# Antibas/eaQHM-analysis-and-synthesis-in-Python

Hardware: AMD Instinct MI355X
Metric: analysis_frames_per_sec (higher is better)
Workload: dtype f64; 1 GPU; synth16k_60s_female_maxAdpt5; samples=960000, fs=16000, ls_frames_per_adaptation=63936, adaptations_executed=5, Kmax=59, track_bytes=906240000, parallelism=instants sharded x1 by LS cost; boundary records all-gathered per adaptation

## Files before the change

eaqhm-analysis-and-synthesis-in-python_amd/csrc/eaqhm_ls_tile.hip:

```cpp
#include <type_traits>
#include "eaqhm_ls_common.h"
#include "eaqhm_ls_chol.h"
#include "eaqhm_ls_a0.h"
#include "eaqhm_ls_tilemap.h"
#include "eaqhm_ls_twunits.h"
#include "eaqhm_ls_gather.h"
#include "eaqhm_ls_tilelds.h"
#include "eaqhm_ls_tilexch.h"

namespace eaqhm {
bool ls_a0tile_fits(const LsArgs& A);
int launch_ls_a0tile(eaqhm_ctx* ctx, LsArgs A);

#define DIAG_OWNER(jb, nt) ((int)TL_DIAG[nt][jb])
#define TL_THREADS 512
#define TL_WAVES 8
#define TL_CW 8
static_assert(TLL_TILE == TL_TILE && TLL_DG_TILE == DG_TILE, "eaqhm_ls_tilelds.h and eaqhm_ls_chol.h disagree");
static_assert(TX_DFLAG_BYTE == 8 * (4 * TL_NTMAX * TL_TILE + 2 * TL_TILE + DGP_DOUBLES + 128 + 256), "eaqhm_ls_tilexch.h: where tile_frame puts dflag");

__device__ inline void fetch_next_header(const LsArgs& A, TlHead* hd, int C, int nbuf, int lane) {
  int* cls = uni(A.cls);
  int item = 0;
  if (lane == 0) item = atomicAdd(cls + 8 + C, 1);
  item = uni(item);
  int f = -1;
  if (item < uni(cls[C])) f = uni(cls[16 + (size_t)C * uni(A.n_frames) + item]);
  if (f >= 0) {
    const int* tab = (lane == 0) ? A.ncol : (lane == 1) ? A.frame_c : (lane == 2) ? A.frame_wl : A.frame_inst;
    if (lane < 4) (&hd->n)[lane] = tab[f];
    const int Kmax = uni(A.Kmax);
    if (lane < TL_NSLOT && lane < Kmax) hd->cols[nbuf][lane] = A.cols[(size_t)f * Kmax + lane];
  }
  if (lane == 0) { hd->f = f; hd->buf = nbuf; hd->cls = C; }
}

__device__ inline void tw_step(d4 (&g)[9], double aR, double aI, double bR, double bI, double nk) {
  const double sA = aR + aI, dB = bI - bR;
  const double naR = nk * aR, naI = nk * aI, nsA = nk * sA;
  const double nbR = nk * bR, nbI = nk * bI, ndB = nk * dB;
  g[0] = __builtin_amdgcn_mfma_f64_16x16x4f64(aR, bR, g[0], 0, 0, 0);
  g[1] = __builtin_amdgcn_mfma_f64_16x16x4f64(aI, bI, g[1], 0, 0, 0);
// ... 45 lines not shown
  g0[0] = __builtin_amdgcn_mfma_f64_16x16x4f64(aR, bR, g0[0], 0, 0, 0);
  g1[0] = __builtin_amdgcn_mfma_f64_16x16x4f64(aR, nbR, g1[0], 0, 0, 0);
  g0[1] = __builtin_amdgcn_mfma_f64_16x16x4f64(aR, bI, g0[1], 0, 0, 0);
  g1[1] = __builtin_amdgcn_mfma_f64_16x16x4f64(aR, nbI, g1[1], 0, 0, 0);
  g0[0] = __builtin_amdgcn_mfma_f64_16x16x4f64(aI, bI, g0[0], 0, 0, 0);
  g1[0] = __builtin_amdgcn_mfma_f64_16x16x4f64(aI, nbI, g1[0], 0, 0, 0);
  g0[1] = __builtin_amdgcn_mfma_f64_16x16x4f64(maI, bR, g0[1], 0, 0, 0);
  g1[1] = __builtin_amdgcn_mfma_f64_16x16x4f64(maI, nbR, g1[1], 0, 0, 0);
}

template <int NS, int TW, int UA = 0, int UB = 0, int TB = 0>
__device__ __attribute__((noinline)) void tile_frame(const LsArgs& A, int TS_, int ldx_max_, double* lds, int f_) {
  constexpr int C = NS == 12 ? 5 : NS == 10 ? 4 : NS == 9 ? 3 : NS == 7 ? 2 : NS == 6 ? 1 : 0;
  static_assert(NS == 12 || NS == 10 || NS == 9 || NS == 7 || NS == 6 || NS == 5, "a register budget per class");
  constexpr bool NEXT_HEAD = NS != 10, REC_ROW = NS == 9;
  const bool pre = uni(f_) < 0;
  const int TS = uni(TS_), ldx_max = uni(ldx_max_);
  const int tid = threadIdx.x, nt_thr = TL_THREADS;
  const int lane = tid & 63;
  const int wave = __builtin_amdgcn_readfirstlane(tid >> 6);
  double* U = uni(lds);
  TlHead* hd = (TlHead*)(U + tl_head_offset());
  const int f = pre ? uni(hd->f) : uni(f_);
  double* Xre = U;
  double* Xim = Xre + (size_t)TS * ldx_max;
  const size_t usize_g = (size_t)2 * TS * ldx_max;
  double* ci = U + usize_g;
  unsigned long long* masks = (unsigned long long*)(ci + (size_t)CI_STRIDE * 52);
  double* PanR = U;
  double* PanI = PanR + TL_NTMAX * TL_TILE;
  double* WtR = PanI + TL_NTMAX * TL_TILE;
  double* WtI = WtR + TL_NTMAX * TL_TILE;
  double* LdR = WtI + TL_NTMAX * TL_TILE;
  double* LdI = LdR + TL_TILE;
  double* Dc = LdI + TL_TILE;
  double* Zc = Dc + DG_TILE;
  double* zv = Zc + DG_TILE;
  double* xv = zv + 2 * 16 * TL_NTMAX;
  double* xs = xv + 32 + TL_HEAD_DOUBLES;
  double* sh = xs + 4 * uni(A.Kcmax);
  double* win = sh + 16;
  double* sig = win + 64 * CI_NCH;
  double* dorig = sig + 64 * CI_NCH;

  const int Npad = ((uni(A.Nmax) + 63) >> 6) << 6;
  double* Qs = uni(A.scratch) + (size_t)blockIdx.x * (size_t)uni((int)A.scratch_stride);
  double* Rs = Qs + (size_t)Npad * uni(A.nmax);
  const bool seeds = uni(hd->seeds) != 0;
  const double w1 = uni(2.0 * M_PI / A.fs);
  const int PE = TS / 2;
  const double* sA = uni(A.s);
  const int lcol = lane & 15, lq = lane >> 4;
  unsigned long long* dbg = uni(A.debug);
  unsigned long long t_prev = 0;

  {
    const int n = pre ? uni(hd->n) : uni(A.ncol[f]);
    const int Kc = 2 * n + 1, Ms = 2 * Kc + 1;
    const int nt = (Ms + 15) >> 4;
    const int c = pre ? uni(hd->c) : uni(A.frame_c[f]), wl = pre ? uni(hd->wl) : uni(A.frame_wl[f]);
    const int inst = pre ? uni(hd->inst) : uni(A.frame_inst[f]);
    const int N = 2 * wl + 1, mid = wl;
    const int T = (Kc + 16) >> 4;
    constexpr int UN = UA + UB;
    constexpr int GA = UA / 3, GB = UB / 3;
    constexpr bool G3 = TW > 0 || UN > 0;
    constexpr bool LDS_XCH = TW > 0;
    static_assert(TW == 0 || UN == 0, "whole pairs or units");
    static_assert(UN == 0 || (UA == TWU_UA && UB == TWU_UB), "slot layout of eaqhm_ls_twunits.h");
    static_assert(TB >= 0 && TB < TWU_NTB, "unit table");
    constexpr bool PK = UN > 0 && TWU_PACKED[TB];
    constexpr int EC = 16 * (TWU_TT[TB] - 1);
    const int nb = G3 ? T : nt;
    const int ldx = (nb << 4) + ((nb & 1) ? 0 : 16);
    const int npair = T * (T + 1) / 2;
    const int is = 2 * Kc - 16 * (nt - 1);
    const double f0 = uni(A.f0_stale);
    const int* mycols = pre ? (const int*)hd->cols[uni(hd->buf)] : uni(A.cols) + (size_t)f * uni(A.Kmax);
    const int npairs = mid + 1;

    if (dbg && tid == 0) {
      t_prev = __builtin_amdgcn_s_memtime();
      if (hd->t_last && !uni((int)A.debug_diag)) atomicAdd(dbg + 11, t_prev - hd->t_last);
    }
    double sv[2];
#pragma unroll
    for (int r = 0; r < 2; ++r) {
      const int t = tid + r * nt_thr;
      sv[r] = (t < N) ? sA[(size_t)(c - wl) + t] : 0.0;
    }
    for (int q = tid; q < TS * ldx; q += nt_thr) { Xre[q] = 0.0; Xim[q] = 0.0; }
#pragma unroll
    for (int r = 0; r < 2; ++r) {
      const int t = tid + r * nt_thr;
      if (t < N) { win[t] = window_value(false, t, N); sig[t] = sv[r]; }
    }
    int* gappy = (int*)(masks + (size_t)52 * CI_NCH);
    prepare_slots<CI_STRIDE, TL_WAVES>(A, Qs, Rs, Npad, ci, masks, gappy, mycols, n, N, mid, c, wl, seeds, lane, wave, CI_NCH,
                                       REC_ROW ? hd->fmc : nullptr);
    LS_STAMP(0);

    constexpr int NM3 = (NS <= 7) ? NS : 0;
    d4 accR[NS], accI[NS], acc3[NM3 ? NM3 : 1];
    int tP[NS], tQ[NS];
    bool live[NS];
#pragma unroll
    for (int sl = 0; sl < NS; ++sl) {
      accR[sl] = (d4){0, 0, 0, 0};
      accI[sl] = (d4){0, 0, 0, 0};
      if (sl < NM3) acc3[sl] = (d4){0, 0, 0, 0};
      const int code = TL_MAP[nt][wave][sl];
      live[sl] = code != 0xFF;
      const int P = live[sl] ? (code >> 4) : 0, Q = live[sl] ? (code & 15) : 0;
      tP[sl] = __builtin_amdgcn_readfirstlane(P);
// ... 12 lines not shown
      gx[sl] = __builtin_amdgcn_readfirstlane(x);
      int I = 0, J = 0;
      if (glive[sl]) tile_of(x, I, J);
      gI[sl] = __builtin_amdgcn_readfirstlane(I);
      gJ[sl] = __builtin_amdgcn_readfirstlane(J);
#pragma unroll
      for (int p = 0; p < 9; ++p) g[sl][p] = (d4){0, 0, 0, 0};
    }

    constexpr int UAA = UA > 3 ? UA : 3, UBA = UB > 3 ? UB : 3;
    d4 ga[UAA][3], gb[UBA][2];
    int ucode[UN ? UN : 1];
    if constexpr (UN > 0) {
#pragma unroll
      for (int sl = 0; sl < UN; ++sl) ucode[sl] = __builtin_amdgcn_readfirstlane((int)TWU_MAPS[TB][wave][sl]);
#pragma unroll
      for (int sl = 0; sl < UA; ++sl)
#pragma unroll
        for (int p = 0; p < 3; ++p) ga[sl][p] = (d4){0, 0, 0, 0};
#pragma unroll
      for (int sl = 0; sl < UB; ++sl) gb[sl][0] = gb[sl][1] = (d4){0, 0, 0, 0};
    }

    for (int d0 = 0; d0 < npairs; d0 += PE) {
#pragma clang loop unroll(disable)
      for (int idx = tid; idx < 16 * n; idx += nt_thr) {
        const int el = idx & 15, j = idx >> 4, d = d0 + el;
        const bool act = d <= mid;
        const int u = mid - d - 1, v = mid + d;
        double su = 0, cu = 1, sv, cv;
        double pur = 0, pui = 0, nur = 0, nui = 0, pvr, pvi, nvr, nvi;
        {
          double* cj = ci + j * CI_STRIDE;
          const double* fb = ((const double**)cj)[2];
          const double* ab = ((const double**)cj)[3];
          const int dc = act ? d : mid;
          const double fu1 = fb[mid - dc], fv = fb[mid + dc];
          const double au = ab[(mid - dc - 1 >= 0) ? (mid - dc - 1) : 0], au1 = ab[mid - dc];
          const double av = ab[mid + dc], av1 = ab[(mid + dc + 1 < N) ? (mid + dc + 1) : (N - 1)];
          const double xu = act ? fu1 : 0.0, xv = (act && d >= 1) ? fv : 0.0;
          const double qv = cj[0] + scan16(xv), qu = -(cj[1] + scan16(xu));
          if (el == 15) { cj[0] = qv; cj[1] = -qu; }
          if (!act) continue;
          const double ainv = cj[17], pr = cj[18], pi = cj[19];
          sincos_cw(qu * w1, &su, &cu);
          sincos_cw(qv * w1, &sv, &cv);
          const double eps = 10e-5;
          if (u >= 0) {
            const double ru = (eps + au) * ainv, rv1 = (eps + av1) * ainv;
            pur = ru * cu;                    pui = ru * su;
            nur = rv1 * (cv * pr - sv * pi);  nui = rv1 * (cv * pi + sv * pr);
          }
          const double rv = (eps + av) * ainv, ru1 = (eps + au1) * ainv;
          pvr = rv * cv;                      pvi = rv * sv;
          nvr = ru1 * (cu * pr - su * pi);    nvi = ru1 * (cu * pi + su * pr);
        }
        double* xr = Xre + (2 * el) * ldx;
        double* xi = Xim + (2 * el) * ldx;
        const int cpos = XCOL(n + 1 + j, el), cneg = XCOL(j, el);
        const int spos = XCOL(Kc + n + 1 + j, el), sneg = XCOL(Kc + j, el);
        const double wv = win[v], nv = (double)(v - mid);
        if (u >= 0) {
          const double wu = win[u], nu = (double)(u - mid);
          pur *= wu; pui *= wu; nur *= wu; nui *= wu;
          xr[cpos] = pur;      xi[cpos] = pui;      xr[cneg] = nur;      xi[cneg] = nui;
          if (!G3) { xr[spos] = nu * pur; xi[spos] = nu * pui; xr[sneg] = nu * nur; xi[sneg] = nu * nui; }
          if (PK && n + 1 + j >= EC) { xr[XCOL(n + 9 + j, el)] = nu * pur; xi[XCOL(n + 9 + j, el)] = nu * pui; }
        }
        pvr *= wv; pvi *= wv; nvr *= wv; nvi *= wv;
        xr += ldx; xi += ldx;
        xr[cpos] = pvr;      xi[cpos] = pvi;      xr[cneg] = nvr;      xi[cneg] = nvi;
        if (!G3) { xr[spos] = nv * pvr; xi[spos] = nv * pvi; xr[sneg] = nv * nvr; xi[sneg] = nv * nvi; }
        if (PK && n + 1 + j >= EC) { xr[XCOL(n + 9 + j, el)] = nv * pvr; xi[XCOL(n + 9 + j, el)] = nv * pvi; }
      }
      if ((tid & 15) == 0 && (tid >> 4) < TS) {
        const int row = tid >> 4;
        const int d = d0 + (row >> 1);
        const int t = (row & 1) ? (mid + d) : (mid - d - 1);
        const bool ok = (d <= mid) && (t >= 0);
        const double w = ok ? win[t] : 0.0;
        const double sval = ok ? sig[t] : 0.0;
        const double nn = (double)(t - mid);
        const int el = row >> 1;
        double* xr = Xre + row * ldx;
        double* xi = Xim + row * ldx;
        xr[XCOL(n, el)] = w;               xi[XCOL(n, el)] = 0.0;
        if (!G3) {
          xr[XCOL(Kc + n, el)] = w * nn;   xi[XCOL(Kc + n, el)] = 0.0;
        }
        const int scol = G3 ? Kc : 2 * Kc;
        xr[XCOL(scol, el)] = w * sval;     xi[XCOL(scol, el)] = 0.0;
        if (PK) { xr[XCOL(Kc + 8, el)] = w * sval * nn;  xi[XCOL(Kc + 8, el)] = 0.0; }
      }
      if (d0 + PE > mid) {
        for (int q = tid; q < TS * 16 * nb; q += nt_thr) {
          const int row = q / (16 * nb), col = q - row * (16 * nb);
          const int d = d0 + (row >> 1);
          const int t = (row & 1) ? (mid + d) : (mid - d - 1);
          if (d > mid || t < 0) { Xre[row * ldx + col] = 0.0; Xim[row * ldx + col] = 0.0; }
        }
      }
      LS_STAMP(12);
      __syncthreads();
      LS_STAMP(1);
      const int pcs = (npairs - d0 < PE) ? (npairs - d0) : PE;
      const int ksl = (pcs + 1) >> 1;
      if constexpr (UN > 0) {
        const int plane = TS * ldx_max;
        const int kn = (ksl < 8) ? ksl : 8;
#pragma unroll
        for (int gi = 0; gi < GA + GB; ++gi) {
          const int s0 = (gi < GA) ? 3 * gi : UA + 3 * (gi - GA);
          const int code = ucode[s0];
          if (code == 0xFFFF) continue;
          const int ca = 16 * ((code >> 8) & 15), cb = 16 * ((code >> 4) & 15);
          const bool k4 = (code & 3) == 1;
          int rb = lq * ldx;
          const int sw0 = lcol + (lq >> 1);
          int nk = (lq & 1) ? d0 + (lq >> 1) : -d0 - (lq >> 1) - 1;
          asm volatile("" : "+v"(rb), "+v"(nk));
          if (PK && gi >= GA) {
            if (code & 0x1000) {
              const int q = (gi >= GA) ? 3 * (gi - GA) : 0;
#pragma clang loop unroll(disable)
              for (int ks = 0; ks < kn; ++ks) {
                const int sw = (sw0 + 2 * ks) & 15;
                const double aR = Xre[rb + ca + sw], aI = Xre[rb + ca + sw + plane];
                const double bR = Xre[rb + cb + sw], bI = Xre[rb + cb + sw + plane];
                rb += 4 * ldx;
                twu_edge_k4(gb[q], gb[q + 1], aR, aI, bR, bI, (double)nk);
                nk += (lq & 1) ? 2 : -2;
              }
              continue;
            }
          }
#pragma clang loop unroll(disable)
          for (int ks = 0; ks < kn; ++ks) {
            const int sw = (sw0 + 2 * ks) & 15;
            const double aR = Xre[rb + ca + sw], aI = Xre[rb + ca + sw + plane];
            const double bR = Xre[rb + cb + sw], bI = Xre[rb + cb + sw + plane];
            rb += 4 * ldx;
            if (gi < GA) {
              const int q = (gi < GA) ? 3 * gi : 0;
              twu_pair_k3(ga[q], ga[q + 1], ga[q + 2], aR, aI, bR, bI, (double)nk);
            } else {
              const int q = (gi >= GA) ? 3 * (gi - GA) : 0;
              twu_pair_2acc(gb[q], gb[q + 1], gb[q + 2], aR, aI, bR, bI, (double)nk, k4);
            }
            nk += (lq & 1) ? 2 : -2;
          }
        }
#pragma unroll
        for (int sl = 0; sl < UN; ++sl) {
          if ((sl < UA) ? (sl < 3 * GA) : (sl - UA < 3 * GB)) continue;
          const int code = ucode[sl];
          if (code == 0xFFFF) continue;
          const int ca = 16 * ((code >> 8) & 15), cb = 16 * ((code >> 4) & 15), up = (code >> 2) & 3;
          const bool k4 = (code & 3) == 1;
          int rb = lq * ldx;
          const int sw0 = lcol + (lq >> 1);
          int nk = (lq & 1) ? d0 + (lq >> 1) : -d0 - (lq >> 1) - 1;
          asm volatile("" : "+v"(rb), "+v"(nk));
          auto run = [&](auto pc) {
            constexpr int P = decltype(pc)::value;
#pragma clang loop unroll(disable)
            for (int ks = 0; ks < kn; ++ks) {
              const int sw = (sw0 + 2 * ks) & 15;
              double aR = Xre[rb + ca + sw], aI = Xre[rb + ca + sw + plane];
              double bR = Xre[rb + cb + sw], bI = Xre[rb + cb + sw + plane];
              rb += 4 * ldx;
              if constexpr (P == 1 || P == 2) { aR *= (double)nk; aI *= (double)nk; }
              if constexpr (P >= 2) { bR *= (double)nk; bI *= (double)nk; }
              nk += (lq & 1) ? 2 : -2;
              if (sl < UA) {
                d4 (&g)[3] = ga[sl < UA ? sl : 0];
                g[0] = __builtin_amdgcn_mfma_f64_16x16x4f64(aR, bR, g[0], 0, 0, 0);
                g[1] = __builtin_amdgcn_mfma_f64_16x16x4f64(aI, bI, g[1], 0, 0, 0);
                g[2] = __builtin_amdgcn_mfma_f64_16x16x4f64(aR + aI, bI - bR, g[2], 0, 0, 0);
              } else {
                d4 (&g)[2] = gb[sl >= UA ? sl - UA : 0];
                g[0] = __builtin_amdgcn_mfma_f64_16x16x4f64(aR, bR, g[0], 0, 0, 0);
                g[1] = __builtin_amdgcn_mfma_f64_16x16x4f64(aR, bI, g[1], 0, 0, 0);
                g[0] = __builtin_amdgcn_mfma_f64_16x16x4f64(aI, bI, g[0], 0, 0, 0);
                if (k4) g[1] = __builtin_amdgcn_mfma_f64_16x16x4f64(-aI, bR, g[1], 0, 0, 0);
              }
            }
          };
          if (up == 0) run(std::integral_constant<int, 0>{});
          else if (PK && (code & 0x1000)) run(std::integral_constant<int, PK ? 3 : 1>{});
          else if (up == 1) run(std::integral_constant<int, 1>{});
          else run(std::integral_constant<int, 2>{});
        }
      } else if constexpr (TW > 0) {
#pragma unroll
        for (int sl = 0; sl < TW; ++sl) {
          if (!glive[sl]) continue;
          const int ca = 16 * gI[sl], cb = 16 * gJ[sl];
          int rb = lq * ldx;
          const int sw0 = lcol + (lq >> 1);
          int nk = (lq & 1) ? d0 + (lq >> 1) : -d0 - (lq >> 1) - 1;
          asm volatile("" : "+v"(rb), "+v"(nk));
          const int plane = TS * ldx_max;
          int kn = (ksl < 8) ? ksl : 8;
          int ks = 0;
          if (split && sl == 1) {
            if (wave & 1) { ks = 4; rb += 16 * ldx; nk += (lq & 1) ? 8 : -8; }
            else kn = (kn < 4) ? kn : 4;
          }
#pragma clang loop unroll(disable)
          for (; ks < kn; ++ks) {
            const int sw = (sw0 + 2 * ks) & 15;
            const double aR = Xre[rb + ca + sw], aI = Xre[rb + ca + sw + plane];
            const double bR = Xre[rb + cb + sw], bI = Xre[rb + cb + sw + plane];
            rb += 4 * ldx;
            tw_step(g[sl], aR, aI, bR, bI, (double)nk);
            nk += (lq & 1) ? 2 : -2;
          }
        }
      } else {
#pragma unroll
        for (int sl = 0; sl < NS; ++sl) {
          if (!live[sl]) continue;
          const int ca = 16 * tP[sl], cb = 16 * tQ[sl];
          int rb = lq * ldx;
          const int sw0 = lcol + (lq >> 1);
          asm volatile("" : "+v"(rb));
          const int plane = TS * ldx_max;
          if (ksl < 8) {
#pragma clang loop unroll(disable)
            for (int ks = 0; ks < ksl; ++ks) {
              const int sw = (sw0 + 2 * ks) & 15;
              const double aR = Xre[rb + ca + sw], aI = Xre[rb + ca + sw + plane];
              const double bR = Xre[rb + cb + sw], bI = Xre[rb + cb + sw + plane];
              rb += 4 * ldx;
              if (sl < NM3) {
                accR[sl] = __builtin_amdgcn_mfma_f64_16x16x4f64(aR, bR, accR[sl], 0, 0, 0);
                acc3[sl < NM3 ? sl : 0] = __builtin_amdgcn_mfma_f64_16x16x4f64(aI, bI, acc3[sl < NM3 ? sl : 0], 0, 0, 0);
                accI[sl] = __builtin_amdgcn_mfma_f64_16x16x4f64(aR + aI, bI - bR, accI[sl], 0, 0, 0);
              } else {
                accR[sl] = __builtin_amdgcn_mfma_f64_16x16x4f64(aR, bR, accR[sl], 0, 0, 0);
                accI[sl] = __builtin_amdgcn_mfma_f64_16x16x4f64(aR, bI, accI[sl], 0, 0, 0);
                accR[sl] = __builtin_amdgcn_mfma_f64_16x16x4f64(aI, bI, accR[sl], 0, 0, 0);
                accI[sl] = __builtin_amdgcn_mfma_f64_16x16x4f64(-aI, bR, accI[sl], 0, 0, 0);
              }
            }
            continue;
          }
          double aR, aI, bR, bI;
          {
            const int sw = sw0 & 15;
            aR = Xre[rb + ca + sw]; aI = Xre[rb + ca + sw + plane]; bR = Xre[rb + cb + sw]; bI = Xre[rb + cb + sw + plane];
          }
#pragma unroll
          for (int ks = 0; ks < 8; ++ks) {
            double naR = 0, naI = 0, nbR = 0, nbI = 0;
            if (ks < 7) {
              rb += 4 * ldx;
              const int sw = (sw0 + 2 * (ks + 1)) & 15;
              naR = Xre[rb + ca + sw]; naI = Xre[rb + ca + sw + plane]; nbR = Xre[rb + cb + sw]; nbI = Xre[rb + cb + sw + plane];
            }
            __builtin_amdgcn_sched_barrier(0);
            if (sl < NM3) {
              accR[sl] = __builtin_amdgcn_mfma_f64_16x16x4f64(aR, bR, accR[sl], 0, 0, 0);
              acc3[sl < NM3 ? sl : 0] = __builtin_amdgcn_mfma_f64_16x16x4f64(aI, bI, acc3[sl < NM3 ? sl : 0], 0, 0, 0);
              accI[sl] = __builtin_amdgcn_mfma_f64_16x16x4f64(aR + aI, bI - bR, accI[sl], 0, 0, 0);
            } else {
              accR[sl] = __builtin_amdgcn_mfma_f64_16x16x4f64(aR, bR, accR[sl], 0, 0, 0);
              accI[sl] = __builtin_amdgcn_mfma_f64_16x16x4f64(aR, bI, accI[sl], 0, 0, 0);
              accR[sl] = __builtin_amdgcn_mfma_f64_16x16x4f64(aI, bI, accR[sl], 0, 0, 0);
              accI[sl] = __builtin_amdgcn_mfma_f64_16x16x4f64(-aI, bR, accI[sl], 0, 0, 0);
            }
            aR = naR; aI = naI; bR = nbR; bI = nbI;
          }
        }
      }
      __syncthreads();
      LS_STAMP(2);
    }
    if constexpr (TW == 0 && NM3 > 0) {
#pragma unroll
      for (int sl = 0; sl < NM3; ++sl) {
        const d4 p1 = accR[sl], p2 = acc3[sl];
        accR[sl] = p1 + p2;
        accI[sl] = accI[sl] + (p1 - p2);
      }
    }
    if constexpr (LDS_XCH) {
      constexpr int PPR = NS == 5 ? 3 : 2, NR = NS == 5 ? 1 : 2;
      static_assert(PPR == tx_planes_per_round(NS == 5 ? 4 : 5) && NR == tx_rounds(NS == 5 ? 4 : 5), "rounds of eaqhm_ls_tilexch.h");
      typedef __attribute__((address_space(3))) char* xch_base_t;
      typedef int xch_i4 __attribute__((ext_vector_type(4)));
      typedef double xch_d2 __attribute__((ext_vector_type(2)));
      typedef __attribute__((address_space(3))) xch_d2* xch_cell_t;
      xch_base_t Xb = (xch_base_t)(char*)U;
      const unsigned tabB = (unsigned)tx_table_byte(uni(A.Kcmax)), zcB = (unsigned)tx_zcell_byte(uni(A.Kcmax));
      const __attribute__((address_space(3))) xch_i4* gtab = (const __attribute__((address_space(3))) xch_i4*)(Xb + tabB);
      if (tid < 16 * nt) {
        const GatherEntry e = gather_entry(tid, Kc, npair, T, false);
        *(__attribute__((address_space(3))) xch_i4*)(Xb + tabB + 32 * tid) = (xch_i4){e.lo, e.hi, e.trow, e.tcol};
      }
// ... 485 lines not shown
  const size_t bridged = 2 * Npad * nmax, gram = (size_t)3 * 21 * 512 + 2;
  return ((bridged > gram ? bridged : gram) + 15) & ~(size_t)15;
}

int launch_ls_prepass(eaqhm_ctx* ctx, LsArgs A, long long track_t0) {
  hipLaunchKernelGGL(eaqhm_ls_classify_kernel, dim3((A.n_frames + 255) / 256), dim3(256), 0, ctx->stream, A);
  HIP_TRY(ctx, hipGetLastError());
  if (A.mode == 1) {
    const int ch0 = (int)(track_t0 >> 10), ch1 = (int)((track_t0 + A.Lt - 1) >> 10);
    hipLaunchKernelGGL(eaqhm_ls_zero_prefix_kernel, dim3(ch1 - ch0 + 1, A.Kmax), dim3(256), 0, ctx->stream, A.fm_cur, A.Lt,
                       track_t0, ch0, A.zchunks, A.zflag, (unsigned short*)A.zloc, (int*)A.ztot);
    HIP_TRY(ctx, hipGetLastError());
  }
  return EAQHM_OK;
}

int launch_ls_tile(eaqhm_ctx* ctx, LsArgs A, int grid) {
  if (A.mode == 0 && ctx->a0_resident && ls_a0tile_fits(A)) return launch_ls_a0tile(ctx, A);
  const int Kcmax = A.Kcmax;
  const int ldx_max = 16 * TL_NTMAX + 16;
  const int TS = 32;
  const size_t lds_bytes = tl_lds_doubles(Kcmax, TS, ldx_max) * sizeof(double);
  if (lds_bytes > TL_LDS_LIMIT) return ctx->fail(EAQHM_EINVAL, "eaqhm_ls_batch: LDS budget exceeded (tile variant)");
  if (!tl_layout_ok(TS, ldx_max)) return ctx->fail(EAQHM_EINVAL, "eaqhm_ls_batch: LDS layout (tile variant)");
  if (a0_lds_doubles(A0_M, 2, TZ_TB, TZ_NCH, 520, 64 * CI_NCH, Kcmax) * sizeof(double) > lds_bytes)
    return ctx->fail(EAQHM_EINVAL, "eaqhm_ls_batch: LDS budget exceeded (adaptation 0, tile variant)");
  HIP_TRY(ctx, hipFuncSetAttribute((const void*)eaqhm_ls_tile_kernel, hipFuncAttributeMaxDynamicSharedMemorySize, (int)lds_bytes));
  hipLaunchKernelGGL(eaqhm_ls_tile_kernel, dim3(grid), dim3(TL_THREADS), lds_bytes, ctx->stream, A, TS, ldx_max);
  HIP_TRY(ctx, hipGetLastError());
  return EAQHM_OK;
}

}
```

eaqhm-analysis-and-synthesis-in-python_amd/csrc/eaqhm_ls_tilelds.h:

```cpp
#pragma once
#include <cstddef>

#if defined(__HIPCC__)
#define TLL_HD __host__ __device__
#else
#define TLL_HD
#endif

#define TL_NTMAX 13
#define CI_STRIDE 20
#define CI_NCH 16
#define TL_NSLOT 52
#define TLL_TILE (16 * 17)
#define TLL_DG_TILE (2 * 16 * 17)
#define TL_LDS_LIMIT (159 * 1024)

#define TL_HEAD_GAP 16
struct TlHead {
  double gap[TL_HEAD_GAP];
  double fmc[TL_NSLOT];
  unsigned long long t_last;
  int cls, f, n, c, wl, inst, buf, seeds;
  int cols[2][TL_NSLOT];
  int even[2];
};
static_assert(sizeof(TlHead) % 16 == 0, "TlHead: a multiple of 16 bytes");
#define TL_HEAD_DOUBLES ((sizeof(TlHead) + 7) / 8)

TLL_HD constexpr inline size_t tl_usize_c() {
  return (size_t)4 * TL_NTMAX * TLL_TILE + 2 * TLL_TILE + 2 * TLL_DG_TILE + 2 * 16 * TL_NTMAX + 32;
}
TLL_HD inline size_t tl_usize_g(int TS, int ldx_max) {
  return (size_t)2 * TS * ldx_max + (size_t)CI_STRIDE * TL_NSLOT + TL_NSLOT * CI_NCH + 32;
}
TLL_HD inline size_t tl_head_offset() { return tl_usize_c(); }
TLL_HD inline bool tl_layout_ok(int TS, int ldx_max) { return tl_usize_g(TS, ldx_max) <= tl_usize_c() + TL_HEAD_GAP; }
TLL_HD inline size_t tl_lds_doubles(int Kcmax, int TS, int ldx_max) {
  const size_t c = tl_usize_c() + TL_HEAD_DOUBLES, g = tl_usize_g(TS, ldx_max);
  return (c > g ? c : g) + 4 * (size_t)Kcmax + 16 + 2 * 64 * CI_NCH + 16 * TL_NTMAX;
}

inline bool tl_applicable(int Kcmax, int Nmax) {
  return Nmax <= 64 * CI_NCH && tl_layout_ok(32, 16 * TL_NTMAX + 16) && tl_lds_doubles(Kcmax, 32, 16 * TL_NTMAX + 16) * sizeof(double) <= TL_LDS_LIMIT;
}
```

Before: 1.711 million frames/s.

## Double-buffer design-matrix chunks so half the waves build while others run MFMA

Adds a double-buffered chunk schedule for the grouped (G3) tile-frame classes selected by a class mask (class 3 by default). The X chunk buffers are split into two halves within the existing LDS plane. Half the waves build the next chunk while the others accumulate MFMA Gram products on the previous one, which leaves one barrier per half-step pair instead of two per chunk. The aim is to overlap the sincos/scan basis construction with the MFMA accumulation. In exchange it zeroes both buffers, adds loop-control overhead, and assigns the build and MFMA phases unevenly to each wave group.

```diff
diff --git a/eaqhm-analysis-and-synthesis-in-python_amd/csrc/eaqhm_ls_tile.hip b/eaqhm-analysis-and-synthesis-in-python_amd/csrc/eaqhm_ls_tile.hip
--- a/eaqhm-analysis-and-synthesis-in-python_amd/csrc/eaqhm_ls_tile.hip
+++ b/eaqhm-analysis-and-synthesis-in-python_amd/csrc/eaqhm_ls_tile.hip
@@ -18,6 +18,13 @@
 #define TL_CW 8
 static_assert(TLL_TILE == TL_TILE && TLL_DG_TILE == DG_TILE, "eaqhm_ls_tilelds.h and eaqhm_ls_chol.h disagree");
 static_assert(TX_DFLAG_BYTE == 8 * (4 * TL_NTMAX * TL_TILE + 2 * TL_TILE + DGP_DOUBLES + 128 + 256), "eaqhm_ls_tilexch.h: where tile_frame puts dflag");
+
+#ifndef EAQHM_CHUNK_SCHED
+#define EAQHM_CHUNK_SCHED 2
+#endif
+#ifndef EAQHM_CHUNK_CLASSES
+#define EAQHM_CHUNK_CLASSES 0x08
+#endif
 
 __device__ inline void fetch_next_header(const LsArgs& A, TlHead* hd, int C, int nbuf, int lane) {
   int* cls = uni(A.cls);
@@ -109,8 +116,8 @@
   double* U = uni(lds);
   TlHead* hd = (TlHead*)(U + tl_head_offset());
   const int f = pre ? uni(hd->f) : uni(f_);
-  double* Xre = U;
-  double* Xim = Xre + (size_t)TS * ldx_max;
+  double* Xre0 = U;
+  double* Xim0 = Xre0 + (size_t)TS * ldx_max;
   const size_t usize_g = (size_t)2 * TS * ldx_max;
   double* ci = U + usize_g;
   unsigned long long* masks = (unsigned long long*)(ci + (size_t)CI_STRIDE * 52);
@@ -153,6 +160,9 @@
     constexpr int GA = UA / 3, GB = UB / 3;
     constexpr bool G3 = TW > 0 || UN > 0;
     constexpr bool LDS_XCH = TW > 0;
+    constexpr bool DBUF = G3 && EAQHM_CHUNK_SCHED > 0 && ((EAQHM_CHUNK_CLASSES >> C) & 1);
+    constexpr bool K2 = DBUF && TW > 0 && EAQHM_CHUNK_SCHED == 3;
+    const int xbuf = (int)tl_chunk_buffer_offset(TS, ldx_max);
     static_assert(TW == 0 || UN == 0, "whole pairs or units");
     static_assert(UN == 0 || (UA == TWU_UA && UB == TWU_UB), "slot layout of eaqhm_ls_twunits.h");
     static_assert(TB >= 0 && TB < TWU_NTB, "unit table");
@@ -176,7 +186,10 @@
       const int t = tid + r * nt_thr;
       sv[r] = (t < N) ? sA[(size_t)(c - wl) + t] : 0.0;
     }
-    for (int q = tid; q < TS * ldx; q += nt_thr) { Xre[q] = 0.0; Xim[q] = 0.0; }
+    for (int q = tid; q < TS * ldx; q += nt_thr) {
+      Xre0[q] = 0.0; Xim0[q] = 0.0;
+      if constexpr (DBUF) { Xre0[q + xbuf] = 0.0; Xim0[q + xbuf] = 0.0; }
+    }
 #pragma unroll
     for (int r = 0; r < 2; ++r) {
       const int t = tid + r * nt_thr;
@@ -235,217 +248,273 @@
       for (int sl = 0; sl < UB; ++sl) gb[sl][0] = gb[sl][1] = (d4){0, 0, 0, 0};
     }
 
-    for (int d0 = 0; d0 < npairs; d0 += PE) {
+    const int nchunk = (npairs + PE - 1) / PE;
+    const int late = EAQHM_CHUNK_SCHED == 1 ? 0 : EAQHM_CHUNK_SCHED == 4 ? (wave & 1) : (wave >> 2);
+    for (int it = 0; it < (DBUF ? 2 * (nchunk + 1) : npairs); it += DBUF ? 1 : PE) {
+      const int s = (it >> 1) - 1, half = it & 1;
+      if (!DBUF || (half == late && s + 1 < nchunk)) {
+        const int d0 = DBUF ? (s + 1) * PE : it;
+        double* const Xre = Xre0 + ((DBUF && (s & 1) == 0) ? xbuf : 0);
+        double* const Xim = Xim0 + ((DBUF && (s & 1) == 0) ? xbuf : 0);
 #pragma clang loop unroll(disable)
-      for (int idx = tid; idx < 16 * n; idx += nt_thr) {
-        const int el = idx & 15, j = idx >> 4, d = d0 + el;
-        const bool act = d <= mid;
-        const int u = mid - d - 1, v = mid + d;
-        double su = 0, cu = 1, sv, cv;
-        double pur = 0, pui = 0, nur = 0, nui = 0, pvr, pvi, nvr, nvi;
-        {
-          double* cj = ci + j * CI_STRIDE;
-          const double* fb = ((const double**)cj)[2];
-          const double* ab = ((const double**)cj)[3];
-          const int dc = act ? d : mid;
-          const double fu1 = fb[mid - dc], fv = fb[mid + dc];
-          const double au = ab[(mid - dc - 1 >= 0) ? (mid - dc - 1) : 0], au1 = ab[mid - dc];
-          const double av = ab[mid + dc], av1 = ab[(mid + dc + 1 < N) ? (mid + dc + 1) : (N - 1)];
-          const double xu = act ? fu1 : 0.0, xv = (act && d >= 1) ? fv : 0.0;
-          const double qv = cj[0] + scan16(xv), qu = -(cj[1] + scan16(xu));
-          if (el == 15) { cj[0] = qv; cj[1] = -qu; }
-          if (!act) continue;
-          const double ainv = cj[17], pr = cj[18], pi = cj[19];
-          sincos_cw(qu * w1, &su, &cu);
-          sincos_cw(qv * w1, &sv, &cv);
-          const double eps = 10e-5;
+        for (int idx = tid; idx < 16 * n; idx += nt_thr) {
+          const int el = idx & 15, j = idx >> 4, d = d0 + el;
+          const bool act = d <= mid;
+          const int u = mid - d - 1, v = mid + d;
+          double su = 0, cu = 1, sv, cv;
+          double pur = 0, pui = 0, nur = 0, nui = 0, pvr, pvi, nvr, nvi;
+          {
+            double* cj = ci + j * CI_STRIDE;
+            const double* fb = ((const double**)cj)[2];
+            const double* ab = ((const double**)cj)[3];
+            const int dc = act ? d : mid;
+            const double fu1 = fb[mid - dc], fv = fb[mid + dc];
+            const double au = ab[(mid - dc - 1 >= 0) ? (mid - dc - 1) : 0], au1 = ab[mid - dc];
+            const double av = ab[mid + dc], av1 = ab[(mid + dc + 1 < N) ? (mid + dc + 1) : (N - 1)];
+            const double xu = act ? fu1 : 0.0, xv = (act && d >= 1) ? fv : 0.0;
+            const double qv = cj[0] + scan16(xv), qu = -(cj[1] + scan16(xu));
+            if (el == 15) { cj[0] = qv; cj[1] = -qu; }
+            if (!act) continue;
+            const double ainv = cj[17], pr = cj[18], pi = cj[19];
+            sincos_cw(qu * w1, &su, &cu);
+            sincos_cw(qv * w1, &sv, &cv);
+            const double eps = 10e-5;
+            if (u >= 0) {
+              const double ru = (eps + au) * ainv, rv1 = (eps + av1) * ainv;
+              pur = ru * cu;                    pui = ru * su;
+              nur = rv1 * (cv * pr - sv * pi);  nui = rv1 * (cv * pi + sv * pr);
+            }
+            const double rv = (eps + av) * ainv, ru1 = (eps + au1) * ainv;
+            pvr = rv * cv;                      pvi = rv * sv;
+            nvr = ru1 * (cu * pr - su * pi);    nvi = ru1 * (cu * pi + su * pr);
+          }
+          double* xr = Xre + (2 * el) * ldx;
+          double* xi = Xim + (2 * el) * ldx;
+          const int cpos = XCOL(n + 1 + j, el), cneg = XCOL(j, el);
+          const int spos = XCOL(Kc + n + 1 + j, el), sneg = XCOL(Kc + j, el);
+          const double wv = win[v], nv = (double)(v - mid);
           if (u >= 0) {
-            const double ru = (eps + au) * ainv, rv1 = (eps + av1) * ainv;
-            pur = ru * cu;                    pui = ru * su;
-            nur = rv1 * (cv * pr - sv * pi);  nui = rv1 * (cv * pi + sv * pr);
-          }
-          const double rv = (eps + av) * ainv, ru1 = (eps + au1) * ainv;
-          pvr = rv * cv;                      pvi = rv * sv;
-          nvr = ru1 * (cu * pr - su * pi);    nvi = ru1 * (cu * pi + su * pr);
-        }
-        double* xr = Xre + (2 * el) * ldx;
-        double* xi = Xim + (2 * el) * ldx;
-        const int cpos = XCOL(n + 1 + j, el), cneg = XCOL(j, el);
-        const int spos = XCOL(Kc + n + 1 + j, el), sneg = XCOL(Kc + j, el);
-        const double wv = win[v], nv = (double)(v - mid);
-        if (u >= 0) {
-          const double wu = win[u], nu = (double)(u - mid);
-          pur *= wu; pui *= wu; nur *= wu; nui *= wu;
-          xr[cpos] = pur;      xi[cpos] = pui;      xr[cneg] = nur;      xi[cneg] = nui;
-          if (!G3) { xr[spos] = nu * pur; xi[spos] = nu * pui; xr[sneg] = nu * nur; xi[sneg] = nu * nui; }
-          if (PK && n + 1 + j >= EC) { xr[XCOL(n + 9 + j, el)] = nu * pur; xi[XCOL(n + 9 + j, el)] = nu * pui; }
-        }
-        pvr *= wv; pvi *= wv; nvr *= wv; nvi *= wv;
-        xr += ldx; xi += ldx;
-        xr[cpos] = pvr;      xi[cpos] = pvi;      xr[cneg] = nvr;      xi[cneg] = nvi;
-        if (!G3) { xr[spos] = nv * pvr; xi[spos] = nv * pvi; xr[sneg] = nv * nvr; xi[sneg] = nv * nvi; }
-        if (PK && n + 1 + j >= EC) { xr[XCOL(n + 9 + j, el)] = nv * pvr; xi[XCOL(n + 9 + j, el)] = nv * pvi; }
-      }
-      if ((tid & 15) == 0 && (tid >> 4) < TS) {
-        const int row = tid >> 4;
-        const int d = d0 + (row >> 1);
-        const int t = (row & 1) ? (mid + d) : (mid - d - 1);
-        const bool ok = (d <= mid) && (t >= 0);
-        const double w = ok ? win[t] : 0.0;
-        const double sval = ok ? sig[t] : 0.0;
-        const double nn = (double)(t - mid);
-        const int el = row >> 1;
-        double* xr = Xre + row * ldx;
-        double* xi = Xim + row * ldx;
-        xr[XCOL(n, el)] = w;               xi[XCOL(n, el)] = 0.0;
-        if (!G3) {
-          xr[XCOL(Kc + n, el)] = w * nn;   xi[XCOL(Kc + n, el)] = 0.0;
-        }
-        const int scol = G3 ? Kc : 2 * Kc;
-        xr[XCOL(scol, el)] = w * sval;     xi[XCOL(scol, el)] = 0.0;
-        if (PK) { xr[XCOL(Kc + 8, el)] = w * sval * nn;  xi[XCOL(Kc + 8, el)] = 0.0; }
-      }
-      if (d0 + PE > mid) {
-        for (int q = tid; q < TS * 16 * nb; q += nt_thr) {
-          const int row = q / (16 * nb), col = q - row * (16 * nb);
+            const double wu = win[u], nu = (double)(u - mid);
+            pur *= wu; pui *= wu; nur *= wu; nui *= wu;
+            xr[cpos] = pur;      xi[cpos] = pui;      xr[cneg] = nur;      xi[cneg] = nui;
+            if (!G3) { xr[spos] = nu * pur; xi[spos] = nu * pui; xr[sneg] = nu * nur; xi[sneg] = nu * nui; }
+            if (PK && n + 1 + j >= EC) { xr[XCOL(n + 9 + j, el)] = nu * pur; xi[XCOL(n + 9 + j, el)] = nu * pui; }
+          }
+          pvr *= wv; pvi *= wv; nvr *= wv; nvi *= wv;
+          xr += ldx; xi += ldx;
+          xr[cpos] = pvr;      xi[cpos] = pvi;      xr[cneg] = nvr;      xi[cneg] = nvi;
+          if (!G3) { xr[spos] = nv * pvr; xi[spos] = nv * pvi; xr[sneg] = nv * nvr; xi[sneg] = nv * nvi; }
+          if (PK && n + 1 + j >= EC) { xr[XCOL(n + 9 + j, el)] = nv * pvr; xi[XCOL(n + 9 + j, el)] = nv * pvi; }
+        }
+        if ((tid & 15) == 0 && (tid >> 4) < TS) {
+          const int row = tid >> 4;
           const int d = d0 + (row >> 1);
           const int t = (row & 1) ? (mid + d) : (mid - d - 1);
-          if (d > mid || t < 0) { Xre[row * ldx + col] = 0.0; Xim[row * ldx + col] = 0.0; }
-        }
-      }
-      LS_STAMP(12);
-      __syncthreads();
-      LS_STAMP(1);
-      const int pcs = (npairs - d0 < PE) ? (npairs - d0) : PE;
-      const int ksl = (pcs + 1) >> 1;
-      if constexpr (UN > 0) {
-        const int plane = TS * ldx_max;
-        const int kn = (ksl < 8) ? ksl : 8;
-#pragma unroll
-        for (int gi = 0; gi < GA + GB; ++gi) {
-          const int s0 = (gi < GA) ? 3 * gi : UA + 3 * (gi - GA);
-          const int code = ucode[s0];
-          if (code == 0xFFFF) continue;
-          const int ca = 16 * ((code >> 8) & 15), cb = 16 * ((code >> 4) & 15);
-          const bool k4 = (code & 3) == 1;
-          int rb = lq * ldx;
-          const int sw0 = lcol + (lq >> 1);
-          int nk = (lq & 1) ? d0 + (lq >> 1) : -d0 - (lq >> 1) - 1;
-          asm volatile("" : "+v"(rb), "+v"(nk));
-          if (PK && gi >= GA) {
-            if (code & 0x1000) {
-              const int q = (gi >= GA) ? 3 * (gi - GA) : 0;
+          const bool ok = (d <= mid) && (t >= 0);
+          const double w = ok ? win[t] : 0.0;
+          const double sval = ok ? sig[t] : 0.0;
+          const double nn = (double)(t - mid);
+          const int el = row >> 1;
+          double* xr = Xre + row * ldx;
+          double* xi = Xim + row * ldx;
+          xr[XCOL(n, el)] = w;               xi[XCOL(n, el)] = 0.0;
+          if (!G3) {
+            xr[XCOL(Kc + n, el)] = w * nn;   xi[XCOL(Kc + n, el)] = 0.0;
+          }
+          const int scol = G3 ? Kc : 2 * Kc;
+          xr[XCOL(scol, el)] = w * sval;     xi[XCOL(scol, el)] = 0.0;
+          if (PK) { xr[XCOL(Kc + 8, el)] = w * sval * nn;  xi[XCOL(Kc + 8, el)] = 0.0; }
+        }
+        if (d0 + PE > mid) {
+          for (int q = tid; q < TS * 16 * nb; q += nt_thr) {
+            const int row = q / (16 * nb), col = q - row * (16 * nb);
+            const int d = d0 + (row >> 1);
+            const int t = (row & 1) ? (mid + d) : (mid - d - 1);
+            if (d > mid || t < 0) { Xre[row * ldx + col] = 0.0; Xim[row * ldx + col] = 0.0; }
+          }
+        }
+      }
+      if constexpr (!DBUF) {
+        LS_STAMP(12);
+        __syncthreads();
+        LS_STAMP(1);
+      } else if (half == 0) {
+        LS_STAMP(12);
+      }
+      if (!DBUF || (half != late && s >= 0)) {
+        const int d0 = DBUF ? s * PE : it;
+        const double* const Xre = Xre0 + ((DBUF && (s & 1)) ? xbuf : 0);
+        const int pcs = (npairs - d0 < PE) ? (npairs - d0) : PE;
+        const int ksl = (pcs + 1) >> 1;
+        if constexpr (UN > 0) {
+          const int plane = TS * ldx_max;
+          const int kn = (ksl < 8) ? ksl : 8;
+#pragma unroll
+          for (int gi = 0; gi < GA + GB; ++gi) {
+            const int s0 = (gi < GA) ? 3 * gi : UA + 3 * (gi - GA);
+            const int code = ucode[s0];
+            if (code == 0xFFFF) continue;
+            const int ca = 16 * ((code >> 8) & 15), cb = 16 * ((code >> 4) & 15);
+            const bool k4 = (code & 3) == 1;
+            int rb = lq * ldx;
+            const int sw0 = lcol + (lq >> 1);
+            int nk = (lq & 1) ? d0 + (lq >> 1) : -d0 - (lq >> 1) - 1;
+            asm volatile("" : "+v"(rb), "+v"(nk));
+            if (PK && gi >= GA) {
+              if (code & 0x1000) {
+                const int q = (gi >= GA) ? 3 * (gi - GA) : 0;
+#pragma clang loop unroll(disable)
+                for (int ks = 0; ks < kn; ++ks) {
+                  const int sw = (sw0 + 2 * ks) & 15;
+                  const double aR = Xre[rb + ca + sw], aI = Xre[rb + ca + sw + plane];
+                  const double bR = Xre[rb + cb + sw], bI = Xre[rb + cb + sw + plane];
+                  rb += 4 * ldx;
+                  twu_edge_k4(gb[q], gb[q + 1], aR, aI, bR, bI, (double)nk);
+                  nk += (lq & 1) ? 2 : -2;
+                }
+                continue;
+              }
+            }
+#pragma clang loop unroll(disable)
+            for (int ks = 0; ks < kn; ++ks) {
+              const int sw = (sw0 + 2 * ks) & 15;
+              const double aR = Xre[rb + ca + sw], aI = Xre[rb + ca + sw + plane];
+              const double bR = Xre[rb + cb + sw], bI = Xre[rb + cb + sw + plane];
+              rb += 4 * ldx;
+              if (gi < GA) {
+                const int q = (gi < GA) ? 3 * gi : 0;
+                twu_pair_k3(ga[q], ga[q + 1], ga[q + 2], aR, aI, bR, bI, (double)nk);
+              } else {
+                const int q = (gi >= GA) ? 3 * (gi - GA) : 0;
+                twu_pair_2acc(gb[q], gb[q + 1], gb[q + 2], aR, aI, bR, bI, (double)nk, k4);
+              }
+              nk += (lq & 1) ? 2 : -2;
+            }
+          }
+#pragma unroll
+          for (int sl = 0; sl < UN; ++sl) {
+            if ((sl < UA) ? (sl < 3 * GA) : (sl - UA < 3 * GB)) continue;
+            const int code = ucode[sl];
+            if (code == 0xFFFF) continue;
+            const int ca = 16 * ((code >> 8) & 15), cb = 16 * ((code >> 4) & 15), up = (code >> 2) & 3;
+            const bool k4 = (code & 3) == 1;
+            int rb = lq * ldx;
+            const int sw0 = lcol + (lq >> 1);
+            int nk = (lq & 1) ? d0 + (lq >> 1) : -d0 - (lq >> 1) - 1;
+            asm volatile("" : "+v"(rb), "+v"(nk));
+            auto run = [&](auto pc) {
+              constexpr int P = decltype(pc)::value;
 #pragma clang loop unroll(disable)
               for (int ks = 0; ks < kn; ++ks) {
+                const int sw = (sw0 + 2 * ks) & 15;
+                double aR = Xre[rb + ca + sw], aI = Xre[rb + ca + sw + plane];
+                double bR = Xre[rb + cb + sw], bI = Xre[rb + cb + sw + plane];
+                rb += 4 * ldx;
+                if constexpr (P == 1 || P == 2) { aR *= (double)nk; aI *= (double)nk; }
+                if constexpr (P >= 2) { bR *= (double)nk; bI *= (double)nk; }
+                nk += (lq & 1) ? 2 : -2;
+                if (sl < UA) {
+                  d4 (&g)[3] = ga[sl < UA ? sl : 0];
+                  g[0] = __builtin_amdgcn_mfma_f64_16x16x4f64(aR, bR, g[0], 0, 0, 0);
+                  g[1] = __builtin_amdgcn_mfma_f64_16x16x4f64(aI, bI, g[1], 0, 0, 0);
+                  g[2] = __builtin_amdgcn_mfma_f64_16x16x4f64(aR + aI, bI - bR, g[2], 0, 0, 0);
+                } else {
+                  d4 (&g)[2] = gb[sl >= UA ? sl - UA : 0];
+                  g[0] = __builtin_amdgcn_mfma_f64_16x16x4f64(aR, bR, g[0], 0, 0, 0);
+                  g[1] = __builtin_amdgcn_mfma_f64_16x16x4f64(aR, bI, g[1], 0, 0, 0);
+                  g[0] = __builtin_amdgcn_mfma_f64_16x16x4f64(aI, bI, g[0], 0, 0, 0);
+                  if (k4) g[1] = __builtin_amdgcn_mfma_f64_16x16x4f64(-aI, bR, g[1], 0, 0, 0);
+                }
+              }
+            };
+            if (up == 0) run(std::integral_constant<int, 0>{});
+            else if (PK && (code & 0x1000)) run(std::integral_constant<int, PK ? 3 : 1>{});
+            else if (up == 1) run(std::integral_constant<int, 1>{});
+            else run(std::integral_constant<int, 2>{});
+          }
+        } else if constexpr (TW > 0) {
+#pragma unroll
+          for (int sl = 0; sl < TW; ++sl) {
+            if (!glive[sl]) continue;
+            const int ca = 16 * gI[sl], cb = 16 * gJ[sl];
+            int rb = lq * ldx;
+            const int sw0 = lcol + (lq >> 1);
+            int nk = (lq & 1) ? d0 + (lq >> 1) : -d0 - (lq >> 1) - 1;
+            asm volatile("" : "+v"(rb), "+v"(nk));
+            const int plane = TS * ldx_max;
+            int kn = (ksl < 8) ? ksl : 8;
+            int ks = 0;
+            if (split && sl == 1) {
+              if (wave & 1) { ks = 4; rb += 16 * ldx; nk += (lq & 1) ? 8 : -8; }
+              else kn = (kn < 4) ? kn : 4;
+            }
+            if constexpr (K2) {
+#pragma clang loop unroll(disable)
+              for (; ks + 1 < kn; ks += 2) {
+                const int sw = (sw0 + 2 * ks) & 15, sx = (sw0 + 2 * ks + 2) & 15, rc = rb + 4 * ldx;
+                const double aR = Xre[rb + ca + sw], aI = Xre[rb + ca + sw + plane];
+                const double bR = Xre[rb + cb + sw], bI = Xre[rb + cb + sw + plane];
+                const double cR = Xre[rc + ca + sx], cI = Xre[rc + ca + sx + plane];
+                const double dR = Xre[rc + cb + sx], dI = Xre[rc + cb + sx + plane];
+                rb += 8 * ldx;
+                tw_step(g[sl], aR, aI, bR, bI, (double)nk);
+                tw_step(g[sl], cR, cI, dR, dI, (double)(nk + ((lq & 1) ? 2 : -2)));
+                nk += (lq & 1) ? 4 : -4;
+              }
+            }
+#pragma clang loop unroll(disable)
+            for (; ks < kn; ++ks) {
+              const int sw = (sw0 + 2 * ks) & 15;
+              const double aR = Xre[rb + ca + sw], aI = Xre[rb + ca + sw + plane];
+              const double bR = Xre[rb + cb + sw], bI = Xre[rb + cb + sw + plane];
+              rb += 4 * ldx;
+              tw_step(g[sl], aR, aI, bR, bI, (double)nk);
+              nk += (lq & 1) ? 2 : -2;
+            }
+          }
+        } else {
+#pragma unroll
+          for (int sl = 0; sl < NS; ++sl) {
+            if (!live[sl]) continue;
+            const int ca = 16 * tP[sl], cb = 16 * tQ[sl];
+            int rb = lq * ldx;
+            const int sw0 = lcol + (lq >> 1);
+            asm volatile("" : "+v"(rb));
+            const int plane = TS * ldx_max;
+            if (ksl < 8) {
+#pragma clang loop unroll(disable)
+              for (int ks = 0; ks < ksl; ++ks) {
                 const int sw = (sw0 + 2 * ks) & 15;
                 const double aR = Xre[rb + ca + sw], aI = Xre[rb + ca + sw + plane];
                 const double bR = Xre[rb + cb + sw], bI = Xre[rb + cb + sw + plane];
                 rb += 4 * ldx;
-                twu_edge_k4(gb[q], gb[q + 1], aR, aI, bR, bI, (double)nk);
-                nk += (lq & 1) ? 2 : -2;
+                if (sl < NM3) {
+                  accR[sl] = __builtin_amdgcn_mfma_f64_16x16x4f64(aR, bR, accR[sl], 0, 0, 0);
+                  acc3[sl < NM3 ? sl : 0] = __builtin_amdgcn_mfma_f64_16x16x4f64(aI, bI, acc3[sl < NM3 ? sl : 0], 0, 0, 0);
+                  accI[sl] = __builtin_amdgcn_mfma_f64_16x16x4f64(aR + aI, bI - bR, accI[sl], 0, 0, 0);
+                } else {
+                  accR[sl] = __builtin_amdgcn_mfma_f64_16x16x4f64(aR, bR, accR[sl], 0, 0, 0);
+                  accI[sl] = __builtin_amdgcn_mfma_f64_16x16x4f64(aR, bI, accI[sl], 0, 0, 0);
+                  accR[sl] = __builtin_amdgcn_mfma_f64_16x16x4f64(aI, bI, accR[sl], 0, 0, 0);
+                  accI[sl] = __builtin_amdgcn_mfma_f64_16x16x4f64(-aI, bR, accI[sl], 0, 0, 0);
+                }
               }
               continue;
             }
-          }
-#pragma clang loop unroll(disable)
-          for (int ks = 0; ks < kn; ++ks) {
-            const int sw = (sw0 + 2 * ks) & 15;
-            const double aR = Xre[rb + ca + sw], aI = Xre[rb + ca + sw + plane];
-            const double bR = Xre[rb + cb + sw], bI = Xre[rb + cb + sw + plane];
-            rb += 4 * ldx;
-            if (gi < GA) {
-              const int q = (gi < GA) ? 3 * gi : 0;
-              twu_pair_k3(ga[q], ga[q + 1], ga[q + 2], aR, aI, bR, bI, (double)nk);
-            } else {
-              const int q = (gi >= GA) ? 3 * (gi - GA) : 0;
-              twu_pair_2acc(gb[q], gb[q + 1], gb[q + 2], aR, aI, bR, bI, (double)nk, k4);
-            }
-            nk += (lq & 1) ? 2 : -2;
-          }
-        }
-#pragma unroll
-        for (int sl = 0; sl < UN; ++sl) {
-          if ((sl < UA) ? (sl < 3 * GA) : (sl - UA < 3 * GB)) continue;
-          const int code = ucode[sl];
-          if (code == 0xFFFF) continue;
-          const int ca = 16 * ((code >> 8) & 15), cb = 16 * ((code >> 4) & 15), up = (code >> 2) & 3;
-          const bool k4 = (code & 3) == 1;
-          int rb = lq * ldx;
-          const int sw0 = lcol + (lq >> 1);
-          int nk = (lq & 1) ? d0 + (lq >> 1) : -d0 - (lq >> 1) - 1;
-          asm volatile("" : "+v"(rb), "+v"(nk));
-          auto run = [&](auto pc) {
-            constexpr int P = decltype(pc)::value;
-#pragma clang loop unroll(disable)
-            for (int ks = 0; ks < kn; ++ks) {
-              const int sw = (sw0 + 2 * ks) & 15;
-              double aR = Xre[rb + ca + sw], aI = Xre[rb + ca + sw + plane];
-              double bR = Xre[rb + cb + sw], bI = Xre[rb + cb + sw + plane];
-              rb += 4 * ldx;
-              if constexpr (P == 1 || P == 2) { aR *= (double)nk; aI *= (double)nk; }
-              if constexpr (P >= 2) { bR *= (double)nk; bI *= (double)nk; }
-              nk += (lq & 1) ? 2 : -2;
-              if (sl < UA) {
-                d4 (&g)[3] = ga[sl < UA ? sl : 0];
-                g[0] = __builtin_amdgcn_mfma_f64_16x16x4f64(aR, bR, g[0], 0, 0, 0);
-                g[1] = __builtin_amdgcn_mfma_f64_16x16x4f64(aI, bI, g[1], 0, 0, 0);
-                g[2] = __builtin_amdgcn_mfma_f64_16x16x4f64(aR + aI, bI - bR, g[2], 0, 0, 0);
-              } else {
-                d4 (&g)[2] = gb[sl >= UA ? sl - UA : 0];
-                g[0] = __builtin_amdgcn_mfma_f64_16x16x4f64(aR, bR, g[0], 0, 0, 0);
-                g[1] = __builtin_amdgcn_mfma_f64_16x16x4f64(aR, bI, g[1], 0, 0, 0);
-                g[0] = __builtin_amdgcn_mfma_f64_16x16x4f64(aI, bI, g[0], 0, 0, 0);
-                if (k4) g[1] = __builtin_amdgcn_mfma_f64_16x16x4f64(-aI, bR, g[1], 0, 0, 0);
+            double aR, aI, bR, bI;
+            {
+              const int sw = sw0 & 15;
+              aR = Xre[rb + ca + sw]; aI = Xre[rb + ca + sw + plane]; bR = Xre[rb + cb + sw]; bI = Xre[rb + cb + sw + plane];
+            }
+#pragma unroll
+            for (int ks = 0; ks < 8; ++ks) {
+              double naR = 0, naI = 0, nbR = 0, nbI = 0;
+              if (ks < 7) {
+                rb += 4 * ldx;
+                const int sw = (sw0 + 2 * (ks + 1)) & 15;
+                naR = Xre[rb + ca + sw]; naI = Xre[rb + ca + sw + plane]; nbR = Xre[rb + cb + sw]; nbI = Xre[rb + cb + sw + plane];
               }
-            }
-          };
-          if (up == 0) run(std::integral_constant<int, 0>{});
-          else if (PK && (code & 0x1000)) run(std::integral_constant<int, PK ? 3 : 1>{});
-          else if (up == 1) run(std::integral_constant<int, 1>{});
-          else run(std::integral_constant<int, 2>{});
-        }
-      } else if constexpr (TW > 0) {
-#pragma unroll
-        for (int sl = 0; sl < TW; ++sl) {
-          if (!glive[sl]) continue;
-          const int ca = 16 * gI[sl], cb = 16 * gJ[sl];
-          int rb = lq * ldx;
-          const int sw0 = lcol + (lq >> 1);
-          int nk = (lq & 1) ? d0 + (lq >> 1) : -d0 - (lq >> 1) - 1;
-          asm volatile("" : "+v"(rb), "+v"(nk));
-          const int plane = TS * ldx_max;
-          int kn = (ksl < 8) ? ksl : 8;
-          int ks = 0;
-          if (split && sl == 1) {
-            if (wave & 1) { ks = 4; rb += 16 * ldx; nk += (lq & 1) ? 8 : -8; }
-            else kn = (kn < 4) ? kn : 4;
-          }
-#pragma clang loop unroll(disable)
-          for (; ks < kn; ++ks) {
-            const int sw = (sw0 + 2 * ks) & 15;
-            const double aR = Xre[rb + ca + sw], aI = Xre[rb + ca + sw + plane];
-            const double bR = Xre[rb + cb + sw], bI = Xre[rb + cb + sw + plane];
-            rb += 4 * ldx;
-            tw_step(g[sl], aR, aI, bR, bI, (double)nk);
-            nk += (lq & 1) ? 2 : -2;
-          }
-        }
-      } else {
-#pragma unroll
-        for (int sl = 0; sl < NS; ++sl) {
-          if (!live[sl]) continue;
-          const int ca = 16 * tP[sl], cb = 16 * tQ[sl];
-          int rb = lq * ldx;
-          const int sw0 = lcol + (lq >> 1);
-          asm volatile("" : "+v"(rb));
-          const int plane = TS * ldx_max;
-          if (ksl < 8) {
-#pragma clang loop unroll(disable)
-            for (int ks = 0; ks < ksl; ++ks) {
-              const int sw = (sw0 + 2 * ks) & 15;
-              const double aR = Xre[rb + ca + sw], aI = Xre[rb + ca + sw + plane];
-              const double bR = Xre[rb + cb + sw], bI = Xre[rb + cb + sw + plane];
-              rb += 4 * ldx;
+              __builtin_amdgcn_sched_barrier(0);
               if (sl < NM3) {
                 accR[sl] = __builtin_amdgcn_mfma_f64_16x16x4f64(aR, bR, accR[sl], 0, 0, 0);
                 acc3[sl < NM3 ? sl : 0] = __builtin_amdgcn_mfma_f64_16x16x4f64(aI, bI, acc3[sl < NM3 ? sl : 0], 0, 0, 0);
@@ -456,39 +525,19 @@
                 accR[sl] = __builtin_amdgcn_mfma_f64_16x16x4f64(aI, bI, accR[sl], 0, 0, 0);
                 accI[sl] = __builtin_amdgcn_mfma_f64_16x16x4f64(-aI, bR, accI[sl], 0, 0, 0);
               }
-            }
-            continue;
-          }
-          double aR, aI, bR, bI;
-          {
-            const int sw = sw0 & 15;
-            aR = Xre[rb + ca + sw]; aI = Xre[rb + ca + sw + plane]; bR = Xre[rb + cb + sw]; bI = Xre[rb + cb + sw + plane];
-          }
-#pragma unroll
-          for (int ks = 0; ks < 8; ++ks) {
-            double naR = 0, naI = 0, nbR = 0, nbI = 0;
-            if (ks < 7) {
-              rb += 4 * ldx;
-              const int sw = (sw0 + 2 * (ks + 1)) & 15;
-              naR = Xre[rb + ca + sw]; naI = Xre[rb + ca + sw + plane]; nbR = Xre[rb + cb + sw]; nbI = Xre[rb + cb + sw + plane];
-            }
-            __builtin_amdgcn_sched_barrier(0);
-            if (sl < NM3) {
-              accR[sl] = __builtin_amdgcn_mfma_f64_16x16x4f64(aR, bR, accR[sl], 0, 0, 0);
-              acc3[sl < NM3 ? sl : 0] = __builtin_amdgcn_mfma_f64_16x16x4f64(aI, bI, acc3[sl < NM3 ? sl : 0], 0, 0, 0);
-              accI[sl] = __builtin_amdgcn_mfma_f64_16x16x4f64(aR + aI, bI - bR, accI[sl], 0, 0, 0);
-            } else {
-              accR[sl] = __builtin_amdgcn_mfma_f64_16x16x4f64(aR, bR, accR[sl], 0, 0, 0);
-              accI[sl] = __builtin_amdgcn_mfma_f64_16x16x4f64(aR, bI, accI[sl], 0, 0, 0);
-              accR[sl] = __builtin_amdgcn_mfma_f64_16x16x4f64(aI, bI, accR[sl], 0, 0, 0);
-              accI[sl] = __builtin_amdgcn_mfma_f64_16x16x4f64(-aI, bR, accI[sl], 0, 0, 0);
-            }
-            aR = naR; aI = naI; bR = nbR; bI = nbI;
-          }
-        }
-      }
-      __syncthreads();
-      LS_STAMP(2);
+              aR = naR; aI = naI; bR = nbR; bI = nbI;
+            }
+          }
+        }
+      }
+      if constexpr (!DBUF) {
+        __syncthreads();
+        LS_STAMP(2);
+      } else if (half == 1) {
+        LS_STAMP(2);
+        __syncthreads();
+        LS_STAMP(1);
+      }
     }
     if constexpr (TW == 0 && NM3 > 0) {
 #pragma unroll
@@ -1020,7 +1069,7 @@
   const int TS = 32;
   const size_t lds_bytes = tl_lds_doubles(Kcmax, TS, ldx_max) * sizeof(double);
   if (lds_bytes > TL_LDS_LIMIT) return ctx->fail(EAQHM_EINVAL, "eaqhm_ls_batch: LDS budget exceeded (tile variant)");
-  if (!tl_layout_ok(TS, ldx_max)) return ctx->fail(EAQHM_EINVAL, "eaqhm_ls_batch: LDS layout (tile variant)");
+  if (!tl_layout_ok(TS, ldx_max) || !tl_chunk_buffers_ok(TS, ldx_max)) return ctx->fail(EAQHM_EINVAL, "eaqhm_ls_batch: LDS layout (tile variant)");
   if (a0_lds_doubles(A0_M, 2, TZ_TB, TZ_NCH, 520, 64 * CI_NCH, Kcmax) * sizeof(double) > lds_bytes)
     return ctx->fail(EAQHM_EINVAL, "eaqhm_ls_batch: LDS budget exceeded (adaptation 0, tile variant)");
   HIP_TRY(ctx, hipFuncSetAttribute((const void*)eaqhm_ls_tile_kernel, hipFuncAttributeMaxDynamicSharedMemorySize, (int)lds_bytes));
diff --git a/eaqhm-analysis-and-synthesis-in-python_amd/csrc/eaqhm_ls_tilelds.h b/eaqhm-analysis-and-synthesis-in-python_amd/csrc/eaqhm_ls_tilelds.h
--- a/eaqhm-analysis-and-synthesis-in-python_amd/csrc/eaqhm_ls_tilelds.h
+++ b/eaqhm-analysis-and-synthesis-in-python_amd/csrc/eaqhm_ls_tilelds.h
@@ -35,6 +35,9 @@
 }
 TLL_HD inline size_t tl_head_offset() { return tl_usize_c(); }
 TLL_HD inline bool tl_layout_ok(int TS, int ldx_max) { return tl_usize_g(TS, ldx_max) <= tl_usize_c() + TL_HEAD_GAP; }
+#define TL_LDX_G3 (16 * 6 + 16)
+TLL_HD inline size_t tl_chunk_buffer_offset(int TS, int ldx_max) { return (size_t)TS * ldx_max / 2; }
+TLL_HD inline bool tl_chunk_buffers_ok(int TS, int ldx_max) { return (size_t)TS * TL_LDX_G3 <= tl_chunk_buffer_offset(TS, ldx_max); }
 TLL_HD inline size_t tl_lds_doubles(int Kcmax, int TS, int ldx_max) {
   const size_t c = tl_usize_c() + TL_HEAD_DOUBLES, g = tl_usize_g(TS, ldx_max);
   return (c > g ? c : g) + 4 * (size_t)Kcmax + 16 + 2 * 64 * CI_NCH + 16 * TL_NTMAX;
```

Result: no change. 1.724 million frames/s (median of 6 runs) (+0.8%).
